# PantoMatrix/PantoMatrix

Hardware: NVIDIA H100
Metric: motion_frames_per_sec (higher is better)
Workload: dtype fp16x3 (two fp16 operand planes, 3 products, f32 accumulate)

## Files before the change

### include/pm_emage.h

```cpp
#ifndef PM_EMAGE_H
#define PM_EMAGE_H
#include <stdint.h>
#ifdef __cplusplus
extern "C" {
#endif

#define PM_ABI_VERSION 5
#define PM_FMT_F16 0x100
int pm_abi_version(void);
int pm_memset_async(void* ptr, int value, long long bytes, void* stream);
int pm_device_cc(void);

int pm_tapgemm_f32(const float* A, long long a_bs, int lda, int batch, int rows_in, int cin,
                   const float* W, const float* bias, int taps, int stride, int pad,
                   int rows_out, int cout,
                   const float* residual, long long r_bs, int ldr,
                   int act, float slope,
                   float* out, long long o_bs, int ldo, void* stream);

int pm_tapgemm_tc(const uint16_t* A, long long a_ps, long long a_bs, int lda, int batch, int rows_in, int cin,
                  const uint16_t* W, long long w_ps, int w_rows, int ldw, int taps, int pad, int nsplit,
                  const float* bias, int rows_out, int cout,
                  const float* residual, long long r_bs, int ldr,
                  int act, int act_cols, float slope, float acc_scale,
                  float* out_f32, long long o_bs, int ldo,
                  uint16_t* out_bf16, long long ob_ps, long long ob_bs, int ldob, int out_nsplit,
                  const void* prefetch, long long prefetch_bytes, void* stream);

int pm_split_bf16(const float* x, long long x_bs, int ldx, int batch, int rows, int ch,
                  uint16_t* out, long long o_ps, long long o_bs, int ldo, int nsplit, void* stream);

int pm_wav_stem_f32(const float* audio, long long a_bs, long long a_ws, int batch, int windows, int n_samples,
                    const float* w1, const float* b1, const float* wd, const float* bd, int cout,
                    int ksize, int stride, int pad, int rows_out, float slope,
                    float* y1, float* sc,
                    uint16_t* planes, long long p_ps, int p_ld, int p_nsplit, void* stream);

int pm_add_layernorm_f32(const float* x, const float* r, const float* gamma, const float* beta,
                         float* out, long long rows, int ch, float eps,
                         uint16_t* planes, long long p_ps, int p_ld, int p_nsplit, void* stream);

int pm_attention_f32(const float* Q, int ldq, const float* K, int ldk, const float* V, int ldv,
                     float* O, int ldo, int batch, int heads, int tq, int tk, int head_dim,
                     uint16_t* planes, long long p_ps, int p_ld, int p_nsplit, void* stream);

int pm_attention_tc(const uint16_t* Q, long long q_ps, long long q_bs, int ldq, int q_cols, int q_col0,
                    const uint16_t* K, long long k_ps, long long k_bs, int ldk, int k_cols, int k_col0,
                    const uint16_t* V, long long v_ps, long long v_bs, int ldv, int v_cols, int v_col0,
                    float* O, int ldo, int batch, int heads, int tq, int tk, int head_dim,
                    uint16_t* planes, long long p_ps, int p_ld, int p_nsplit, void* stream);

int pm_add_rows_f32(const float* x, const float* pe, const float* spk, int first, int second,
                    float* out, int batch, int rows, int ch,
                    uint16_t* planes, long long p_ps, int p_ld, int p_nsplit, void* stream);
int pm_add2_f32(const float* a, const float* b, float* out, long long n, int ch,
                uint16_t* planes, long long p_ps, int p_ld, int p_nsplit, void* stream);
int pm_add2_strided_f32(const float* a, long long lda, const float* b, long long ldb, float* out, long long ldo,
                        long long rows, long long ch,
                        uint16_t* planes, long long p_ps, int p_ld, int p_nsplit, void* stream);

int pm_window_input_f32(const float* motion, const float* mask, const float* seed, const float* mask_embedding,
                        float* out, int batch, int total_len, int start, int win_len, int pre, int ch, long long seed_bs,
                        uint16_t* planes, long long p_ps, int p_ld, int p_nsplit, void* stream);

int pm_l2_argmin_f32(const float* z, long long rows, int rows_per_batch, long long z_bs,
                     const float* codebook, const float* e2, int n_codes, int e_dim, long long* index, void* stream);
int pm_l2_argmin_tc(const float* z, long long rows, int rows_per_batch, long long z_bs,
                    const float* codebook, const float* e2, int n_codes, int e_dim, long long* index, int max_ctas,
                    void* stream);
int pm_l2_argmin_simt_f32(const float* z, long long rows, int rows_per_batch, long long z_bs,
                          const float* codebook, const float* e2, int n_codes, int e_dim, long long* index, void* stream);
int pm_row_argmax_f32(const float* x, long long rows, int ch, int ldx, int rows_per_batch, long long x_bs,
                      long long* index, int* nonfinite, void* stream);
int pm_gather_rows_f32(const float* codebook, long long n_table, const long long* index, long long rows, int ch,
                       float* out, uint16_t* planes, long long p_ps, int p_ld, int p_nsplit, void* stream);
int pm_row_sqnorm_f32(const float* x, int rows, int ch, float* out, void* stream);

int pm_pose_compose_f32(const float* face, const float* upper, const float* hands, const float* lower,
                        float* expression, float* axis_angle, float* motion4inf, long long bt, void* stream);

int pm_global_trans_f32(const float* rec, int ld, int vel_off, const float* ref_trans, int ref_bs, float dt,
                        float* trans, int batch, int t, void* stream);

int pm_resample_poly_f32(const void* pcm, int is_int16, long long in_bs, int batch, long long n_in, int channels,
                         const float* bank, int up, int down, int taps, long long n_pre_remove,
                         float* out, long long out_bs, void* stream);

int pm_lstm_bidir_f32(const float* xproj, long long x_bs, int ldx, const float* whh,
                      float* y, long long y_bs, int ldy, unsigned int* barrier,
                      int batch, int t, int hidden, void* stream);
int pm_lstm_cond_f32(const float* spk, long long n_spk, int spk_dim, const long long* speaker_id,
// ... 11 lines not shown
```

### pantomatrix_b200/csrc/pm_tapgemm_tc.cu

```cuda
#include <cuda.h>
#include <stdio.h>
#include <stdlib.h>

#include <cstring>
#include "pm_common.cuh"
#include "../../include/pm_emage.h"


namespace {

constexpr int BM = 128;
constexpr int BK = 64;
constexpr int MMA_K = 16;
constexpr int A_TILE_BYTES = BM * BK * 2;
constexpr int CONSUMER_THREADS = 256;
constexpr int NUM_THREADS = CONSUMER_THREADS + 32;
constexpr int MAX_STAGES = 8;
constexpr int RING_KB = 200;

struct TcParams {
  int taps, pad, nsplit, kblocks;
  int rows_out, cout, batch;
  int R, NB;
  int w_rows;
  const float* bias;
  const float* residual; long long r_bs; int ldr;
  int act, act_cols; float slope;
  float* out_f32; long long o_bs; int ldo;
  __nv_bfloat16* out_bf16; long long ob_ps, ob_bs; int ldob; int out_nsplit;
  int stages;
  const uint8_t* prefetch; long long prefetch_bytes;
  float acc_scale;
};

#ifdef PM_TC_TIMING
__device__ unsigned long long pm_tc_stamps[4096 * 8];
#define PM_STAMP(i)                                                                                              \
  do {                                                                                                           \
    if ((threadIdx.x & 31) == 0) {                                                                               \
      const unsigned cta_ = (blockIdx.z * gridDim.y + blockIdx.y) * gridDim.x + blockIdx.x;                      \
      if (cta_ < 4096) pm_tc_stamps[cta_ * 8 + (i)] = (unsigned long long)clock64();                             \
    }                                                                                                            \
  } while (0)
#else
#define PM_STAMP(i) do {} while (0)
#endif

#include "pm_tc_ptx.cuh"

template <int BN, bool F16>
__device__ __forceinline__ void mma_k16(float (&d)[BN / 2], uint64_t a, uint64_t b) {
  static_assert(BN == 64, "64-column tiles (see pm_tapgemm_tc)");
  wgmma_m64n64k16<!F16>(d, a, b);
}

template <int BN, bool F16, int NSPLIT>
__device__ __forceinline__ void mma_kblock(float (&main)[BN / 2], float (&corr)[BN / 2], uint64_t a0, uint64_t w0) {
  constexpr uint64_t A_PL = A_TILE_BYTES >> 4, W_PL = (BN * BK * 2) >> 4, K_ST = (MMA_K * 2) >> 4;
  if constexpr (NSPLIT == 3) {
#pragma unroll
    for (int k = 0; k < BK / MMA_K; ++k) mma_k16<BN, F16>(corr, a0 + k * K_ST, w0 + 2 * W_PL + k * K_ST);
#pragma unroll
    for (int k = 0; k < BK / MMA_K; ++k) mma_k16<BN, F16>(corr, a0 + A_PL + k * K_ST, w0 + W_PL + k * K_ST);
#pragma unroll
    for (int k = 0; k < BK / MMA_K; ++k) mma_k16<BN, F16>(corr, a0 + 2 * A_PL + k * K_ST, w0 + k * K_ST);
  }
  if constexpr (NSPLIT >= 2) {
#pragma unroll
    for (int k = 0; k < BK / MMA_K; ++k) mma_k16<BN, F16>(corr, a0 + k * K_ST, w0 + W_PL + k * K_ST);
#pragma unroll
    for (int k = 0; k < BK / MMA_K; ++k) mma_k16<BN, F16>(corr, a0 + A_PL + k * K_ST, w0 + k * K_ST);
  }
#pragma unroll
  for (int k = 0; k < BK / MMA_K; ++k) mma_k16<BN, F16>(main, a0 + k * K_ST, w0 + k * K_ST);
}

template <int BN, bool F16, int NSPLIT>
__global__ void __launch_bounds__(NUM_THREADS, 1) tapgemm_tc_kernel(const __grid_constant__ CUtensorMap map_a,
                                                                  const __grid_constant__ CUtensorMap map_w,
                                                                  const TcParams p) {
  constexpr int W_TILE_BYTES = BN * BK * 2;
  constexpr int NACC = BN / 2;
  constexpr int ST = BN + 8;

  extern __shared__ __align__(1024) uint8_t smem_raw[];
  uint8_t* tiles = reinterpret_cast<uint8_t*>((reinterpret_cast<uintptr_t>(smem_raw) + 1023) & ~uintptr_t(1023));
  const int stage_bytes = p.nsplit * (A_TILE_BYTES + W_TILE_BYTES);
  const int ring_bytes = p.stages * stage_bytes > BM * ST * 4 ? p.stages * stage_bytes : BM * ST * 4;
  uint64_t* bars = reinterpret_cast<uint64_t*>(tiles + ring_bytes);
  uint64_t* full_bar = bars;
  uint64_t* empty_bar = bars + MAX_STAGES;

  const int warp = threadIdx.x >> 5, lane = threadIdx.x & 31;
  if (warp == 0) PM_STAMP(0);
  const int l0 = blockIdx.x * p.R;
  const int n0 = blockIdx.y * BN;
  const int b0 = blockIdx.z * p.NB;
  const int n_iter = p.taps * p.kblocks;

  if (threadIdx.x == CONSUMER_THREADS) {
    asm volatile("prefetch.tensormap [%0];" ::"l"(&map_a) : "memory");
    asm volatile("prefetch.tensormap [%0];" ::"l"(&map_w) : "memory");
    for (int s = 0; s < p.stages; ++s) {
      mbar_init(smem_u32(&full_bar[s]), 1);
      mbar_init(smem_u32(&empty_bar[s]), 2);
    }
    asm volatile("fence.mbarrier_init.release.cluster;" ::: "memory");
  }
  __syncthreads();
  if (warp == 0) PM_STAMP(1);

  if (warp == CONSUMER_THREADS / 32) {
    if (lane == 1 && p.prefetch) {
      const long long ncta = (long long)gridDim.x * gridDim.y * gridDim.z;
      const long long cta = ((long long)blockIdx.z * gridDim.y + blockIdx.y) * gridDim.x + blockIdx.x;
      long long share = ((p.prefetch_bytes + ncta - 1) / ncta + 127) & ~127LL;
      long long off = cta * share;
      long long end = off + share < p.prefetch_bytes ? off + share : p.prefetch_bytes;
      end &= ~15LL;
      for (; off < end; off += 16384) {
        const uint32_t n = (uint32_t)(end - off < 16384 ? end - off : 16384);
        asm volatile("cp.async.bulk.prefetch.L2.global [%0], %1;" ::"l"(p.prefetch + off), "r"(n) : "memory");
      }
    }
    __syncwarp();
    const uint32_t tx = (uint32_t)stage_bytes;
    int s = 0, tap = 0, kb = 0;
    uint32_t ph = 0;
    for (int it = 0; it < n_iter; ++it) {
      mbar_wait_fast(smem_u32(&empty_bar[s]), ph ^ 1u);
      if (elect_one()) {
        const uint32_t bar = smem_u32(&full_bar[s]);
        uint8_t* st = tiles + (size_t)s * stage_bytes;
        mbar_expect_tx(bar, tx);
        for (int pl = 0; pl < p.nsplit; ++pl) {
          tma_load_4d(smem_u32(st + pl * A_TILE_BYTES), &map_a, bar, kb * BK, l0 + tap - p.pad, b0, pl);
          tma_load_3d(smem_u32(st + p.nsplit * A_TILE_BYTES + pl * W_TILE_BYTES), &map_w, bar, kb * BK, tap * p.w_rows + n0, pl);
        }
      }
      __syncwarp();
      if (++s == p.stages) { s = 0; ph ^= 1u; }
      if (++kb == p.kblocks) { kb = 0; ++tap; }
    }
    return;
  }

  const int wg = threadIdx.x >> 7;
  float acc0[NACC], acc1[NACC], accc[NACC];
#pragma unroll
  for (int i = 0; i < NACC; ++i) { acc0[i] = 0.f; acc1[i] = 0.f; accc[i] = 0.f; }
  {
    const uint32_t tiles_u32 = smem_u32(tiles);
    int s = 0;
    uint32_t ph = 0;
    int prev = -1;
    auto kblock = [&](float (&main)[NACC]) {
      mbar_wait_fast(smem_u32(&full_bar[s]), ph);
      if (prev < 0 && warp == 0) PM_STAMP(2);
      const uint32_t a_base = tiles_u32 + (uint32_t)s * (uint32_t)stage_bytes + (uint32_t)wg * (64 * 128);
      const uint32_t w_base = tiles_u32 + (uint32_t)s * (uint32_t)stage_bytes + (uint32_t)(NSPLIT * A_TILE_BYTES);
      wgmma_fence();
      mma_kblock<BN, F16, NSPLIT>(main, accc, gmma_desc(GMMA_DESC_K_SW128, a_base), gmma_desc(GMMA_DESC_K_SW128, w_base));
      wgmma_commit();
      wgmma_wait<1>();
      if (prev >= 0 && threadIdx.x % 128 == 0) mbar_arrive(smem_u32(&empty_bar[prev]));
      prev = s;
      if (++s == p.stages) { s = 0; ph ^= 1u; }
    };
    int it = 0;
    for (; it + 1 < n_iter; it += 2) {
      kblock(acc0);
      kblock(acc1);
    }
    if (it < n_iter) kblock(acc0);
    if (warp == 0) PM_STAMP(3);
    wgmma_wait<0>();
    if (warp == 0) PM_STAMP(4);
    wgmma_fence_regs(acc0);
    wgmma_fence_regs(acc1);
    wgmma_fence_regs(accc);
  }
  named_bar_sync(1, CONSUMER_THREADS);
  {
    const int wq = (threadIdx.x >> 5) & 3, t4 = lane & 3;
    const int r0 = wg * 64 + wq * 16 + (lane >> 2);
    float* stg = reinterpret_cast<float*>(tiles);
#pragma unroll
    for (int i = 0; i < NACC / 4; ++i) {
      const int c = 8 * i + 2 * t4;
#pragma unroll
      for (int h = 0; h < 2; ++h) {
        float v0 = acc0[4 * i + 2 * h] + acc1[4 * i + 2 * h];
        float v1 = acc0[4 * i + 2 * h + 1] + acc1[4 * i + 2 * h + 1];
        v0 += accc[4 * i + 2 * h];
        v1 += accc[4 * i + 2 * h + 1];
        if constexpr (F16) { v0 *= p.acc_scale; v1 *= p.acc_scale; }
        *reinterpret_cast<float2*>(stg + (r0 + 8 * h) * ST + c) = make_float2(v0, v1);
      }
    }
  }
  named_bar_sync(1, CONSUMER_THREADS);

  const bool vec_f = p.out_f32 && ((p.ldo & 3) == 0) && ((reinterpret_cast<uintptr_t>(p.out_f32) & 15) == 0) && ((p.o_bs & 3) == 0);
  const bool vec_r = p.residual && ((p.ldr & 3) == 0) && ((reinterpret_cast<uintptr_t>(p.residual) & 15) == 0) && ((p.r_bs & 3) == 0);
  const bool vec_b = p.out_bf16 && ((p.ldob & 3) == 0) && ((reinterpret_cast<uintptr_t>(p.out_bf16) & 7) == 0) &&
                     ((p.ob_bs & 3) == 0) && ((p.ob_ps & 3) == 0);
  const bool all_vec = (!p.out_f32 || vec_f) && (!p.residual || vec_r) && (!p.out_bf16 || vec_b);
  const float act_slope = p.act == PM_ACT_NONE ? 1.f : (p.act == PM_ACT_RELU ? 0.f : p.slope);
  const int r_shift = 31 - __clz(p.R);
  constexpr int C4 = BN / 4;
  const float* stg = reinterpret_cast<const float*>(tiles);
#pragma unroll 1
  for (int item = threadIdx.x; item < BM * C4; item += CONSUMER_THREADS) {
    const int rt = item / C4, c = (item % C4) * 4;
    const int b = b0 + (rt >> r_shift), l = l0 + (rt & (p.R - 1));
    const int n = n0 + c;
    if (b >= p.batch || l >= p.rows_out || n >= p.cout) continue;
    const float4 x4 = *reinterpret_cast<const float4*>(stg + rt * ST + c);
    const long long of = (long long)b * p.o_bs + (long long)l * p.ldo;
    const long long orr = (long long)b * p.r_bs + (long long)l * p.ldr;
    const PmPlanes P{p.out_bf16 ? p.out_bf16 + (long long)b * p.ob_bs + (long long)l * p.ldob : nullptr,
                     p.ob_ps, p.ldob, p.out_nsplit};
    if (all_vec && n + 4 <= p.cout) {
      float4 x = x4;
      if (p.bias) { x.x += __ldg(p.bias + n); x.y += __ldg(p.bias + n + 1); x.z += __ldg(p.bias + n + 2); x.w += __ldg(p.bias + n + 3); }
      if (p.residual) {
        const float4 t = *reinterpret_cast<const float4*>(p.residual + orr + n);
        x.x += t.x; x.y += t.y; x.z += t.z; x.w += t.w;
      }
      x.x = x.x < 0.f ? (n < p.act_cols ? act_slope : 1.f) * x.x : x.x;
      x.y = x.y < 0.f ? (n + 1 < p.act_cols ? act_slope : 1.f) * x.y : x.y;
      x.z = x.z < 0.f ? (n + 2 < p.act_cols ? act_slope : 1.f) * x.z : x.z;
      x.w = x.w < 0.f ? (n + 3 < p.act_cols ? act_slope : 1.f) * x.w : x.w;
      if (p.out_f32) *reinterpret_cast<float4*>(p.out_f32 + of + n) = x;
      if (P.ptr) pm_store_planes4_t<F16>(P, 0, n, x);
    } else {
      const float xs[4] = {x4.x, x4.y, x4.z, x4.w};
#pragma unroll
      for (int k = 0; k < 4; ++k) {
        if (n + k >= p.cout) break;
        float y = xs[k];
        if (p.bias) y += __ldg(p.bias + n + k);
        if (p.residual) y += p.residual[orr + n + k];
        y = y < 0.f ? (n + k < p.act_cols ? act_slope : 1.f) * y : y;
        if (p.out_f32) p.out_f32[of + n + k] = y;
        if (P.ptr) pm_store_planes_t<F16>(P, 0, n + k, y);
      }
    }
  }
  if (warp == 0) PM_STAMP(5);
#ifdef PM_TC_TIMING
  named_bar_sync(1, CONSUMER_THREADS);
#endif
  if (warp == 0) PM_STAMP(6);
}

template <bool VEC, bool F16>
__global__ void __launch_bounds__(256) split_bf16_kernel(const float* __restrict__ x, long long x_bs, int ldx, int rows,
                                                         int ch, __nv_bfloat16* __restrict__ out, long long o_ps,
                                                         long long o_bs, int ldo, int nsplit) {
  const int b = blockIdx.y;
  const float* __restrict__ xb = x + (long long)b * x_bs;
  __nv_bfloat16* __restrict__ ob = out + (long long)b * o_bs;
  if (VEC) {
    const int ch4 = ch >> 2;
    const long long total = (long long)rows * ch4;
    for (long long i = (long long)blockIdx.x * blockDim.x + threadIdx.x; i < total; i += (long long)gridDim.x * blockDim.x) {
      const int r = (int)(i / ch4), c4 = (int)(i - (long long)r * ch4);
      const float4 v = *reinterpret_cast<const float4*>(xb + (long long)r * ldx + 4 * c4);
      const PmPlanes P{ob, o_ps, ldo, nsplit};
      pm_store_planes4_t<F16>(P, r, 4 * c4, v);
    }
  } else {
    const long long total = (long long)rows * ch;
    for (long long i = (long long)blockIdx.x * blockDim.x + threadIdx.x; i < total; i += (long long)gridDim.x * blockDim.x) {
      const int r = (int)(i / ch), c = (int)(i - (long long)r * ch);
      const PmPlanes P{ob, o_ps, ldo, nsplit};
      pm_store_planes_t<F16>(P, r, c, xb[(long long)r * ldx + c]);
    }
  }
}

template <int BN, bool F16, int NSPLIT>
int launch(const CUtensorMap& ma, const CUtensorMap& mw, TcParams& p, dim3 grid, cudaStream_t st) {
  const int stage_bytes = p.nsplit * (A_TILE_BYTES + BN * BK * 2);
  int stages = RING_KB * 1024 / stage_bytes;
  if (stages > MAX_STAGES) stages = MAX_STAGES;
  if (stages < 2) return PM_EUNSUPPORTED;
  p.stages = stages;
  const int staging = BM * (BN + 8) * 4;
  const size_t ring = (size_t)stages * stage_bytes > (size_t)staging ? (size_t)stages * stage_bytes : (size_t)staging;
  const size_t smem = ring + 1024  + 2 * MAX_STAGES * sizeof(uint64_t);
  static unsigned long long configured = 0;
  if (pm_first_use_on_device(configured)) {
    cudaError_t e = cudaFuncSetAttribute(tapgemm_tc_kernel<BN, F16, NSPLIT>, cudaFuncAttributeMaxDynamicSharedMemorySize, 227 * 1024);
    if (e != cudaSuccess) { configured = 0; return (int)e; }
  }
  tapgemm_tc_kernel<BN, F16, NSPLIT><<<grid, NUM_THREADS, smem, st>>>(ma, mw, p);
  PM_LAUNCH_CHECK();
}

}

extern "C" int pm_tapgemm_tc(const uint16_t* A, long long a_ps, long long a_bs, int lda, int batch, int rows_in, int cin,
                             const uint16_t* W, long long w_ps, int w_rows, int ldw, int taps, int pad, int nsplit,
                             const float* bias, int rows_out, int cout,
                             const float* residual, long long r_bs, int ldr,
                             int act, int act_cols, float slope, float acc_scale,
                             float* out_f32, long long o_bs, int ldo,
                             uint16_t* out_bf16, long long ob_ps, long long ob_bs, int ldob, int out_nsplit,
                             const void* prefetch, long long prefetch_bytes, void* stream) {
  PM_REQUIRE(A && W && (out_f32 || out_bf16));
  PM_TAKE_FMT(nsplit, f16);
  PM_TAKE_FMT(out_nsplit, out_f16);
  PM_REQUIRE(!out_bf16 || out_f16 == f16);
  PM_REQUIRE(f16 || acc_scale == 1.0f);
  PM_REQUIRE(!prefetch || (prefetch_bytes >= 0 && (reinterpret_cast<uintptr_t>(prefetch) & 15) == 0));
  PM_REQUIRE(batch > 0 && rows_in > 0 && rows_out > 0 && cin > 0 && cout > 0 && taps > 0);
  PM_REQUIRE(nsplit >= 1 && nsplit <= 3 && (!out_bf16 || (out_nsplit >= 1 && out_nsplit <= 3)));
  PM_REQUIRE(act >= PM_ACT_NONE && act <= PM_ACT_LEAKY);
  PM_REQUIRE((reinterpret_cast<uintptr_t>(A) & 15) == 0 && (reinterpret_cast<uintptr_t>(W) & 15) == 0);
  PM_REQUIRE((lda & 7) == 0 && (ldw & 7) == 0 && lda >= cin && ldw >= cin && w_rows >= cout);
  PM_REQUIRE(batch == 1 || (a_bs & 7) == 0);
  PM_REQUIRE(nsplit == 1 || ((a_ps & 7) == 0 && (w_ps & 7) == 0));
  PM_REQUIRE(!out_f32 || ldo >= cout);
  PM_REQUIRE(!out_bf16 || ldob >= cout);
  PM_REQUIRE(!residual || ldr >= cout);

  int R = 128;
  if (rows_out <= 64 && batch > 1) { R = 16; while (R < rows_out) R <<= 1; }
  const int NB = 128 / R;
  constexpr int BNsel = 64;
  PM_REQUIRE(w_rows % BNsel == 0);

  TcParams p;
  p.taps = taps; p.pad = pad; p.nsplit = nsplit; p.kblocks = (cin + BK - 1) / BK;
  p.rows_out = rows_out; p.cout = cout; p.batch = batch; p.R = R; p.NB = NB; p.w_rows = w_rows;
  p.bias = bias; p.residual = residual; p.r_bs = r_bs; p.ldr = ldr;
  p.act = act; p.act_cols = act_cols <= 0 ? cout : act_cols; p.slope = slope;
  p.out_f32 = out_f32; p.o_bs = o_bs; p.ldo = ldo;
  p.out_bf16 = reinterpret_cast<__nv_bfloat16*>(out_bf16); p.ob_ps = ob_ps; p.ob_bs = ob_bs; p.ldob = ldob;
  p.out_nsplit = out_bf16 ? out_nsplit : 0;
  p.stages = 0;
  p.prefetch = static_cast<const uint8_t*>(prefetch);
  p.prefetch_bytes = prefetch ? prefetch_bytes : 0;
  p.acc_scale = acc_scale;
  CUtensorMap ma, mw;
  {
    const long long bs_el = batch > 1 ? a_bs : (long long)rows_in * lda;
    const long long ps_el = nsplit > 1 ? a_ps : bs_el * batch;
    cuuint64_t dims[4] = {(cuuint64_t)cin, (cuuint64_t)rows_in, (cuuint64_t)batch, (cuuint64_t)nsplit};
    cuuint64_t strides[3] = {(cuuint64_t)lda * 2, (cuuint64_t)bs_el * 2, (cuuint64_t)ps_el * 2};
    cuuint32_t box[4] = {(cuuint32_t)BK, (cuuint32_t)R, (cuuint32_t)NB, 1};
    if (!encode_map(&ma, A, 4, dims, strides, box, f16)) return PM_EBADARG;
  }
  {
    const long long ps_el = nsplit > 1 ? w_ps : (long long)taps * w_rows * ldw;
    cuuint64_t dims[3] = {(cuuint64_t)cin, (cuuint64_t)taps * w_rows, (cuuint64_t)nsplit};
    cuuint64_t strides[2] = {(cuuint64_t)ldw * 2, (cuuint64_t)ps_el * 2};
    cuuint32_t box[3] = {(cuuint32_t)BK, (cuuint32_t)BNsel, 1};
    if (!encode_map(&mw, W, 3, dims, strides, box, f16)) return PM_EBADARG;
  }
  dim3 grid(pm_cdiv(rows_out, R), pm_cdiv(cout, BNsel), pm_cdiv(batch, NB));
  PM_REQUIRE(grid.z <= 65535 && grid.y <= 65535);
  const cudaStream_t st = (cudaStream_t)stream;
  if (f16) {
    if (nsplit == 1) return launch<BNsel, true, 1>(ma, mw, p, grid, st);
    if (nsplit == 2) return launch<BNsel, true, 2>(ma, mw, p, grid, st);
    return launch<BNsel, true, 3>(ma, mw, p, grid, st);
  }
  if (nsplit == 1) return launch<BNsel, false, 1>(ma, mw, p, grid, st);
  if (nsplit == 2) return launch<BNsel, false, 2>(ma, mw, p, grid, st);
  return launch<BNsel, false, 3>(ma, mw, p, grid, st);
}

#ifdef PM_TC_TIMING
extern "C" int pm_tc_timing_reset() {
  cudaError_t e = cudaDeviceSynchronize();
  if (e != cudaSuccess) return (int)e;
  void* d = nullptr;
  e = cudaGetSymbolAddress(&d, pm_tc_stamps);
  if (e != cudaSuccess) return (int)e;
  return (int)cudaMemset(d, 0, sizeof(unsigned long long) * 4096 * 8);
}
extern "C" int pm_tc_timing_read(unsigned long long* host) {
  cudaError_t e = cudaDeviceSynchronize();
  if (e != cudaSuccess) return (int)e;
  return (int)cudaMemcpyFromSymbol(host, pm_tc_stamps, sizeof(unsigned long long) * 4096 * 8);
}
#endif

extern "C" int pm_split_bf16(const float* x, long long x_bs, int ldx, int batch, int rows, int ch,
                             uint16_t* out, long long o_ps, long long o_bs, int ldo, int nsplit, void* stream) {
  PM_TAKE_FMT(nsplit, f16);
  PM_REQUIRE(x && out && batch >= 0 && rows >= 0 && ch > 0 && ldx >= ch && ldo >= ch && nsplit >= 1 && nsplit <= 3);
  if ((long long)batch * rows == 0) return PM_OK;
  PM_REQUIRE(batch <= 65535);
  const bool vec = (ch & 3) == 0 && (ldx & 3) == 0 && (x_bs & 3) == 0 && (ldo & 3) == 0 && (o_bs & 3) == 0 &&
                   (o_ps & 3) == 0 && (reinterpret_cast<uintptr_t>(x) & 15) == 0 && (reinterpret_cast<uintptr_t>(out) & 7) == 0;
  const long long work = (long long)rows * (vec ? ch / 4 : ch);
  long long gx = (work + 255) / 256;
  const long long cap = batch >= 132 * 4 ? 1 : (132 * 8 + batch - 1) / batch;
  if (gx > cap) gx = cap;
  dim3 grid((unsigned)gx, batch);
  __nv_bfloat16* o = reinterpret_cast<__nv_bfloat16*>(out);
  cudaStream_t st = (cudaStream_t)stream;
  if (f16) {
    if (vec) split_bf16_kernel<true, true><<<grid, 256, 0, st>>>(x, x_bs, ldx, rows, ch, o, o_ps, o_bs, ldo, nsplit);
    else split_bf16_kernel<false, true><<<grid, 256, 0, st>>>(x, x_bs, ldx, rows, ch, o, o_ps, o_bs, ldo, nsplit);
  } else {
    if (vec) split_bf16_kernel<true, false><<<grid, 256, 0, st>>>(x, x_bs, ldx, rows, ch, o, o_ps, o_bs, ldo, nsplit);
    else split_bf16_kernel<false, false><<<grid, 256, 0, st>>>(x, x_bs, ldx, rows, ch, o, o_ps, o_bs, ldo, nsplit);
  }
  PM_LAUNCH_CHECK();
}
```

### pantomatrix_b200/csrc/pm_tc_ptx.cuh

```cuda
#pragma once
#include <cuda.h>
#include <stdint.h>

__device__ __forceinline__ uint32_t smem_u32(const void* p) { return (uint32_t)__cvta_generic_to_shared(p); }

__device__ __forceinline__ void mbar_init(uint32_t bar, uint32_t count) {
  asm volatile("mbarrier.init.shared::cta.b64 [%0], %1;" ::"r"(bar), "r"(count) : "memory");
}
__device__ __forceinline__ void mbar_expect_tx(uint32_t bar, uint32_t bytes) {
  asm volatile("mbarrier.arrive.expect_tx.shared::cta.b64 _, [%0], %1;" ::"r"(bar), "r"(bytes) : "memory");
}
__device__ __forceinline__ void mbar_wait(uint32_t bar, uint32_t parity) {
  uint32_t spins = 0;
  long long t0 = 0;
  while (true) {
    uint32_t done;
    asm volatile(
        "{\n\t.reg .pred p;\n\t"
        "mbarrier.try_wait.parity.shared::cta.b64 p, [%1], %2;\n\t"
        "selp.u32 %0, 1, 0, p;\n\t}"
        : "=r"(done) : "r"(bar), "r"(parity) : "memory");
    if (done) return;
    if ((++spins & 0xFFFu) == 0) {
      const long long t = clock64();
      if (t0 == 0) t0 = t;
      else if (t - t0 > 4000000000LL) __trap();
    }
  }
}
template <int SLEEP_NS = 40>
__device__ __forceinline__ void mbar_wait_relaxed(uint32_t bar, uint32_t parity) {
  uint32_t spins = 0;
  while (true) {
    uint32_t done;
    asm volatile(
        "{\n\t.reg .pred p;\n\t"
        "mbarrier.try_wait.parity.shared::cta.b64 p, [%1], %2;\n\t"
        "selp.u32 %0, 1, 0, p;\n\t}"
        : "=r"(done) : "r"(bar), "r"(parity) : "memory");
    if (done) return;
    __nanosleep(SLEEP_NS);
    if (++spins > 50000000u) __trap();
  }
}
__device__ __forceinline__ void mbar_wait_fast(uint32_t bar, uint32_t parity) {
  uint32_t done;
  asm volatile(
      "{\n\t.reg .pred p;\n\t"
      "mbarrier.try_wait.parity.shared::cta.b64 p, [%1], %2;\n\t"
      "selp.u32 %0, 1, 0, p;\n\t}"
      : "=r"(done) : "r"(bar), "r"(parity) : "memory");
  if (!done) mbar_wait(bar, parity);
}
__device__ __forceinline__ bool elect_one() {
  uint32_t pred;
  asm volatile("{\n\t.reg .pred P1;\n\telect.sync _|P1, 0xffffffff;\n\tselp.u32 %0, 1, 0, P1;\n\t}" : "=r"(pred));
  return pred != 0;
}
__device__ __forceinline__ void tma_load_4d(uint32_t dst, const CUtensorMap* map, uint32_t bar, int c0, int c1, int c2, int c3) {
  asm volatile(
      "cp.async.bulk.tensor.4d.shared::cluster.global.mbarrier::complete_tx::bytes [%0], [%1, {%3, %4, %5, %6}], [%2];"
      ::"r"(dst), "l"(map), "r"(bar), "r"(c0), "r"(c1), "r"(c2), "r"(c3) : "memory");
}
__device__ __forceinline__ void tma_load_3d(uint32_t dst, const CUtensorMap* map, uint32_t bar, int c0, int c1, int c2) {
  asm volatile(
      "cp.async.bulk.tensor.3d.shared::cluster.global.mbarrier::complete_tx::bytes [%0], [%1, {%3, %4, %5}], [%2];"
      ::"r"(dst), "l"(map), "r"(bar), "r"(c0), "r"(c1), "r"(c2) : "memory");
}
__device__ __forceinline__ void sts128(uint32_t addr, float a, float b, float c, float d) {
  asm volatile("st.shared.v4.f32 [%0], {%1, %2, %3, %4};" ::"r"(addr), "f"(a), "f"(b), "f"(c), "f"(d) : "memory");
}
__device__ __forceinline__ float4 lds128(uint32_t addr) {
  float4 v;
  asm volatile("ld.shared.v4.f32 {%0, %1, %2, %3}, [%4];" : "=f"(v.x), "=f"(v.y), "=f"(v.z), "=f"(v.w) : "r"(addr) : "memory");
  return v;
}
__device__ __forceinline__ void mbar_arrive(uint32_t bar) {
  asm volatile("mbarrier.arrive.shared::cta.b64 _, [%0];" ::"r"(bar) : "memory");
}
__device__ __forceinline__ void fence_proxy_async_smem() { asm volatile("fence.proxy.async.shared::cta;" ::: "memory"); }
__device__ __forceinline__ float4 ldg_stream4(const float4* p) {
  float4 v;
  asm volatile("ld.global.nc.L1::no_allocate.v4.f32 {%0, %1, %2, %3}, [%4];"
               : "=f"(v.x), "=f"(v.y), "=f"(v.z), "=f"(v.w) : "l"(p));
  return v;
}
__device__ __forceinline__ void named_bar_sync(uint32_t id, uint32_t threads) {
  asm volatile("bar.sync %0, %1;" ::"r"(id), "r"(threads) : "memory");
}

__device__ __forceinline__ void wgmma_fence() { asm volatile("wgmma.fence.sync.aligned;" ::: "memory"); }
__device__ __forceinline__ void wgmma_commit() { asm volatile("wgmma.commit_group.sync.aligned;" ::: "memory"); }
template <int N>
__device__ __forceinline__ void wgmma_wait() { asm volatile("wgmma.wait_group.sync.aligned %0;" ::"n"(N) : "memory"); }
template <int R>
__device__ __forceinline__ void wgmma_fence_regs(float (&d)[R]) {
#pragma unroll
  for (int i = 0; i < R; ++i) asm volatile("" : "+f"(d[i])::"memory");
}
constexpr uint64_t GMMA_DESC_K_SW128 = (1ull << 62) | ((uint64_t)(1024 >> 4) << 32) | (1ull << 16);
constexpr uint64_t gmma_desc_mn_sw128(uint32_t lbo_bytes) {
  return (1ull << 62) | ((uint64_t)(1024 >> 4) << 32) | ((uint64_t)(lbo_bytes >> 4) << 16);
}
__device__ __forceinline__ uint64_t gmma_desc(uint64_t hi, uint32_t smem_addr) { return hi | (uint64_t)((smem_addr >> 4) & 0x3FFFu); }

#define PM_D8(i) "+f"(d[i]), "+f"(d[i + 1]), "+f"(d[i + 2]), "+f"(d[i + 3]), "+f"(d[i + 4]), "+f"(d[i + 5]), "+f"(d[i + 6]), "+f"(d[i + 7])
#define PM_WGMMA_N64(TY)                                                                                   \
  asm volatile("{\n\t.reg .pred p;\n\tsetp.ne.b32 p, %34, 0;\n\t"                                           \
               "wgmma.mma_async.sync.aligned.m64n64k16.f32." TY "." TY " {%0, %1, %2, %3, %4, %5, %6, %7, %8, %9, %10, %11, %12, %13, %14, %15, %16, %17, %18, %19, %20, %21, %22, %23, %24, %25, %26, %27, %28, %29, %30, %31}, %32, %33, p, 1, 1, 0, %35;\n\t}" \
               : PM_D8(0), PM_D8(8), PM_D8(16), PM_D8(24) \
               : "l"(da), "l"(db), "r"(1), "n"(TRANS_B))
template <bool BF16, int TRANS_B = 0>
__device__ __forceinline__ void wgmma_m64n64k16(float (&d)[32], uint64_t da, uint64_t db) {
  if constexpr (BF16) PM_WGMMA_N64("bf16");
  else PM_WGMMA_N64("f16");
}
#undef PM_WGMMA_N64
#define PM_WGMMA_N192(TY)                                                                                   \
  asm volatile("{\n\t.reg .pred p;\n\tsetp.ne.b32 p, %98, 0;\n\t"                                           \
               "wgmma.mma_async.sync.aligned.m64n192k16.f32." TY "." TY " {%0, %1, %2, %3, %4, %5, %6, %7, %8, %9, %10, %11, %12, %13, %14, %15, %16, %17, %18, %19, %20, %21, %22, %23, %24, %25, %26, %27, %28, %29, %30, %31, %32, %33, %34, %35, %36, %37, %38, %39, %40, %41, %42, %43, %44, %45, %46, %47, %48, %49, %50, %51, %52, %53, %54, %55, %56, %57, %58, %59, %60, %61, %62, %63, %64, %65, %66, %67, %68, %69, %70, %71, %72, %73, %74, %75, %76, %77, %78, %79, %80, %81, %82, %83, %84, %85, %86, %87, %88, %89, %90, %91, %92, %93, %94, %95}, %96, %97, p, 1, 1, 0, %99;\n\t}" \
               : PM_D8(0), PM_D8(8), PM_D8(16), PM_D8(24), PM_D8(32), PM_D8(40), PM_D8(48), PM_D8(56), PM_D8(64), PM_D8(72), PM_D8(80), PM_D8(88) \
               : "l"(da), "l"(db), "r"(1), "n"(TRANS_B))
template <bool BF16, int TRANS_B = 0>
__device__ __forceinline__ void wgmma_m64n192k16(float (&d)[96], uint64_t da, uint64_t db) {
  if constexpr (BF16) PM_WGMMA_N192("bf16");
  else PM_WGMMA_N192("f16");
}
#undef PM_WGMMA_N192
#define PM_WGMMA_N256(TY)                                                                                   \
  asm volatile("{\n\t.reg .pred p;\n\tsetp.ne.b32 p, %130, 0;\n\t"                                           \
               "wgmma.mma_async.sync.aligned.m64n256k16.f32." TY "." TY " {%0, %1, %2, %3, %4, %5, %6, %7, %8, %9, %10, %11, %12, %13, %14, %15, %16, %17, %18, %19, %20, %21, %22, %23, %24, %25, %26, %27, %28, %29, %30, %31, %32, %33, %34, %35, %36, %37, %38, %39, %40, %41, %42, %43, %44, %45, %46, %47, %48, %49, %50, %51, %52, %53, %54, %55, %56, %57, %58, %59, %60, %61, %62, %63, %64, %65, %66, %67, %68, %69, %70, %71, %72, %73, %74, %75, %76, %77, %78, %79, %80, %81, %82, %83, %84, %85, %86, %87, %88, %89, %90, %91, %92, %93, %94, %95, %96, %97, %98, %99, %100, %101, %102, %103, %104, %105, %106, %107, %108, %109, %110, %111, %112, %113, %114, %115, %116, %117, %118, %119, %120, %121, %122, %123, %124, %125, %126, %127}, %128, %129, p, 1, 1, 0, %131;\n\t}" \
               : PM_D8(0), PM_D8(8), PM_D8(16), PM_D8(24), PM_D8(32), PM_D8(40), PM_D8(48), PM_D8(56), PM_D8(64), PM_D8(72), PM_D8(80), PM_D8(88), PM_D8(96), PM_D8(104), PM_D8(112), PM_D8(120) \
               : "l"(da), "l"(db), "r"(1), "n"(TRANS_B))
template <bool BF16, int TRANS_B = 0>
__device__ __forceinline__ void wgmma_m64n256k16(float (&d)[128], uint64_t da, uint64_t db) {
  if constexpr (BF16) PM_WGMMA_N256("bf16");
  else PM_WGMMA_N256("f16");
}
#undef PM_WGMMA_N256
#undef PM_D8

typedef CUresult (*EncodeTiledFn)(CUtensorMap*, CUtensorMapDataType, cuuint32_t, void*, const cuuint64_t*,
                                  const cuuint64_t*, const cuuint32_t*, const cuuint32_t*, CUtensorMapInterleave,
                                  CUtensorMapSwizzle, CUtensorMapL2promotion, CUtensorMapFloatOOBfill);

static inline EncodeTiledFn get_encode() {
  static EncodeTiledFn fn = nullptr;
  if (!fn) {
    void* sym = nullptr;
    cudaDriverEntryPointQueryResult q;
    if (cudaGetDriverEntryPoint("cuTensorMapEncodeTiled", &sym, cudaEnableDefault, &q) == cudaSuccess &&
        q == cudaDriverEntryPointSuccess)
      fn = reinterpret_cast<EncodeTiledFn>(sym);
  }
  return fn;
}

static inline bool encode_map(CUtensorMap* m, const void* base, int rank, const cuuint64_t* dims, const cuuint64_t* strides_bytes,
                const cuuint32_t* box, bool f16 = false) {
  EncodeTiledFn fn = get_encode();
  if (!fn) return false;
  cuuint32_t ones[5] = {1, 1, 1, 1, 1};
  return fn(m, f16 ? CU_TENSOR_MAP_DATA_TYPE_FLOAT16 : CU_TENSOR_MAP_DATA_TYPE_BFLOAT16, (cuuint32_t)rank,
            const_cast<void*>(base), dims, strides_bytes, box, ones, CU_TENSOR_MAP_INTERLEAVE_NONE,
            CU_TENSOR_MAP_SWIZZLE_128B, CU_TENSOR_MAP_L2_PROMOTION_L2_256B,
            CU_TENSOR_MAP_FLOAT_OOB_FILL_NONE) == CUDA_SUCCESS;
}
```

### pantomatrix_b200/ops.py

```python
from __future__ import annotations

import math

import torch

from . import _lib

ACT_NONE, ACT_RELU, ACT_LEAKY = 0, 1, 2
ROW_NONE, ROW_PE, ROW_SPK = 0, 1, 2

launch_count = 0

FMT_F16 = 0x100
F16_ACT_SCALE = 64.0
_PLANE_DTYPE = torch.bfloat16


def set_plane_format(name: str) -> None:
    global _PLANE_DTYPE
    _PLANE_DTYPE = {"bf16": torch.bfloat16, "fp16": torch.float16}[name]


def plane_format() -> str:
    return "fp16" if _PLANE_DTYPE == torch.float16 else "bf16"


def _fmt_bit(t) -> int:
    return FMT_F16 if t.dtype == torch.float16 else 0


def _stream() -> int:
    return torch.cuda.current_stream().cuda_stream


def _ptr(t) -> int | None:
    return None if t is None else t.data_ptr()


def _chk(t: torch.Tensor, dtype=torch.float32):
    if not t.is_cuda:
        raise _lib.PmError("pantomatrix_b200 ops need CUDA tensors (no CPU fallback)")
    if t.dtype != dtype:
        raise _lib.PmError(f"expected {dtype}, got {t.dtype}")
    if t.dim() and t.stride(-1) != 1 and t.shape[-1] != 1:
        raise _lib.PmError("innermost dimension must be contiguous")
    return t


def _call(name, *args):
    global launch_count
    launch_count += 1
    _lib.call(name, *args)


def _bs_ld(t: torch.Tensor):
    return (t.stride(0) if t.shape[0] > 1 else t.shape[1] * t.stride(1)), t.stride(1)


def tapgemm(a, w, bias, *, rows_out=None, stride=1, pad=0, act=ACT_NONE, slope=0.0, residual=None, out=None):
    _chk(a), _chk(w)
    batch, rows_in, cin = a.shape
    taps, cout, cin_w = w.shape
    assert cin_w == cin and w.is_contiguous(), (w.shape, a.shape)
    if rows_out is None:
        rows_out = (rows_in + 2 * pad - taps) // stride + 1
    if out is None:
        out = torch.empty(batch, rows_out, cout, device=a.device, dtype=torch.float32)
    else:
        assert out.shape == (batch, rows_out, cout), (out.shape, (batch, rows_out, cout))
    _chk(out)
    if residual is not None:
        _chk(residual)
        assert residual.shape == out.shape
    if (taps == 1 and pad == 0 and stride == 1 and batch > 1 and a.stride(0) == rows_in * a.stride(1)
            and out.stride(0) == rows_out * out.stride(1)
            and (residual is None or residual.stride(0) == rows_out * residual.stride(1))):
        a = a.reshape(1, batch * rows_in, cin) if a.is_contiguous() else a.as_strided(
            (1, batch * rows_in, cin), (0, a.stride(1), 1), a.storage_offset())
        flat = lambda t: t.as_strided((1, batch * rows_out, cout), (0, t.stride(1), 1), t.storage_offset())
        out_v = flat(out)
        res_v = flat(residual) if residual is not None else None
        batch_k, rows_in_k, rows_out_k = 1, batch * rows_in, batch * rows_out
    else:
        out_v, res_v, batch_k, rows_in_k, rows_out_k = out, residual, batch, rows_in, rows_out
    a_bs, lda = _bs_ld(a)
    o_bs, ldo = _bs_ld(out_v)
    r_bs, ldr = _bs_ld(res_v) if res_v is not None else (0, 0)
    _call("pm_tapgemm_f32", a.data_ptr(), a_bs, lda, batch_k, rows_in_k, cin,
          w.data_ptr(), _ptr(bias), taps, stride, pad, rows_out_k, cout,
          _ptr(res_v), r_bs, ldr, act, float(slope), out_v.data_ptr(), o_bs, ldo, _stream())
    return out


def wav_stem(audio, a_bs, a_ws, batch, windows, n_samples, w1, b1, wd, bd, *, stride, pad, slope, offset=0, nsplit=0):
    _chk(audio)
    cout, ks = w1.shape
# ... 261 lines not shown
    expression = torch.empty(bs, t, 100, device=device, dtype=torch.float32)
    axis_angle = torch.empty(bs, t, 165, device=device, dtype=torch.float32)
    motion4inf = torch.empty(bs, t, 337, device=device, dtype=torch.float32)
    _call("pm_pose_compose_f32", _ptr(face), _ptr(upper), _ptr(hands), _ptr(lower), expression.data_ptr(),
          axis_angle.data_ptr(), motion4inf.data_ptr(), bs * t, _stream())
    return expression, axis_angle, motion4inf


def global_trans(rec, ref_trans, dt, vel_off=54):
    _chk(rec), _chk(ref_trans)
    assert rec.is_contiguous()
    bs, t, ld = rec.shape
    assert ref_trans.shape == (bs, 3)
    trans = torch.empty(bs, t, 3, device=rec.device, dtype=torch.float32)
    _call("pm_global_trans_f32", rec.data_ptr(), ld, vel_off, ref_trans.data_ptr(), ref_trans.stride(0), float(dt),
          trans.data_ptr(), bs, t, _stream())
    return trans




def _round_up(x, m):
    return (x + m - 1) // m * m


class Planes:
    __slots__ = ("t", "rows", "ch", "slack")

    def __init__(self, t, rows, ch, slack=0):
        self.t, self.rows, self.ch, self.slack = t, rows, ch, slack

    def flat(self):
        ns, b, r, ld = self.t.shape
        assert self.t.stride(1) == r * self.t.stride(2)
        return Planes(self.t.as_strided((ns, 1, b * r, ld), (self.t.stride(0), b * r * self.t.stride(2), self.t.stride(2), 1),
                                        self.t.storage_offset()), b * r, self.ch, self.slack)

    @property
    def nsplit(self):
        return self.t.shape[0]

    @property
    def batch(self):
        return self.t.shape[1]


def split_bf16(x, nsplit, slack_rows=0):
    _chk(x)
    batch, rows, ch = x.shape
    pl = _new_planes(nsplit, (batch, rows), ch, x.device, slack_rows)
    x_bs, ldx = _bs_ld(x)
    _call("pm_split_bf16", x.data_ptr(), x_bs, ldx, batch, rows, ch, pl.t.data_ptr(), pl.t.stride(0), pl.t.stride(1),
          pl.t.stride(2), nsplit | _fmt_bit(pl.t), _stream())
    return pl


class PackedW:
    __slots__ = ("t", "taps", "cout", "cin", "w_rows", "ldw", "acc_scale")

    def __init__(self, w, nsplit):
        taps, cout, cin = w.shape
        bn = 64 if cout <= 64 else 128
        self.taps, self.cout, self.cin = taps, cout, cin
        self.w_rows, self.ldw = _round_up(cout, bn), _round_up(cin, 8)
        full = torch.zeros(taps, self.w_rows, self.ldw, device=w.device, dtype=torch.float32)
        full[:, :cout, :cin] = w
        self.acc_scale = 1.0
        if _PLANE_DTYPE == torch.float16:
            m = float(full.abs().max())
            if m > 0.0 and math.isfinite(m):
                k = math.floor(math.log2(32768.0 / m))
                full = full * (2.0 ** k)
                self.acc_scale = 2.0 ** -k
            self.acc_scale /= F16_ACT_SCALE
        planes, rem = [], full
        for _ in range(nsplit):
            p = rem.to(_PLANE_DTYPE)
            planes.append(p)
            rem = rem - p.float()
        self.t = torch.stack(planes).contiguous()


def tapgemm_tc(a: Planes, w: PackedW, bias, *, rows_in=None, rows_out, pad=0, act=ACT_NONE, act_cols=0, slope=0.0,
               residual=None, want_f32=True, out_nsplit=0, out=None, a_view=None, out_slack=0, prefetch=None):
    t = a.t
    nsplit, batch = t.shape[0], t.shape[1]
    assert nsplit == w.t.shape[0] and t.dtype == w.t.dtype, "A and W must use the same split and plane format"
    fmt = _fmt_bit(t)
    rows_a, cin, lda = (a.rows, a.ch, t.stride(2)) if a_view is None else a_view
    if rows_in is not None:
        rows_a = rows_in
    assert cin == w.cin, (cin, w.cin)
    cout = w.cout
    dev = t.device
    out_f = None
    if want_f32:
        out_f = out if out is not None else torch.empty(batch, rows_out, cout, device=dev, dtype=torch.float32)
        assert out_f.shape == (batch, rows_out, cout)
    o_bs, ldo = _bs_ld(out_f) if out_f is not None else (0, 0)
    out_p = None
    if out_nsplit:
        out_p = _new_planes(out_nsplit, (batch, rows_out), cout, dev, out_slack, dtype=t.dtype)
    r_bs, ldr = _bs_ld(residual) if residual is not None else (0, 0)
    if residual is not None:
        _chk(residual)
        assert residual.shape == (batch, rows_out, cout)
    _call("pm_tapgemm_tc", t.data_ptr(), t.stride(0), t.stride(1), lda, batch, rows_a, cin,
          w.t.data_ptr(), w.t.stride(0), w.w_rows, w.ldw, w.taps, pad, nsplit | fmt,
          _ptr(bias), rows_out, cout, _ptr(residual), r_bs, ldr, act, act_cols, float(slope), float(w.acc_scale),
          _ptr(out_f), o_bs, ldo,
          None if out_p is None else out_p.t.data_ptr(), 0 if out_p is None else out_p.t.stride(0),
          0 if out_p is None else out_p.t.stride(1), 0 if out_p is None else out_p.t.stride(2),
          out_nsplit | (fmt if out_nsplit else 0),
          None if prefetch is None else prefetch.data_ptr(),
          0 if prefetch is None else prefetch.numel() * prefetch.element_size(), _stream())
    return out_f, out_p




def lstm_bidir(xproj, whh, barrier, hidden):
    _chk(xproj), _chk(whh)
    assert xproj.is_contiguous() and whh.is_contiguous() and whh.shape == (2, 4 * hidden, hidden)
    batch, t, w = xproj.shape
    assert w == 8 * hidden
    y = torch.empty(batch, t, 2 * hidden, device=xproj.device, dtype=torch.float32)
    _call("pm_lstm_bidir_f32", xproj.data_ptr(), xproj.stride(0), xproj.stride(1), whh.data_ptr(), y.data_ptr(),
          y.stride(0), y.stride(1), barrier.data_ptr(), batch, t, hidden, _stream())
    return y


def rot6d_to_aa(rot6d, slot, n_sel):
    _chk(rot6d)
    assert rot6d.is_contiguous() and rot6d.shape[-1] == n_sel * 6
    rows = rot6d.numel() // (n_sel * 6)
    out = torch.empty(*rot6d.shape[:-1], 165, device=rot6d.device, dtype=torch.float32)
    _call("pm_rot6d_to_aa_f32", rot6d.data_ptr(), rows, n_sel, slot.data_ptr(), out.data_ptr(), _stream())
    return out


def softmax2_mix(sel, c1, c2, out=None):
    _chk(sel), _chk(c1), _chk(c2)
    assert sel.is_contiguous() and c1.is_contiguous() and c2.is_contiguous() and sel.shape[-1] == 2
    ch = c1.shape[-1]
    rows = c1.numel() // ch
    if out is None:
        out = torch.empty_like(c1)
    _call("pm_softmax2_mix_f32", sel.data_ptr(), c1.data_ptr(), c2.data_ptr(), out.data_ptr(), rows, ch, out.stride(-2), _stream())
    return out
```

Before: 277,400.

## Add 128-column wgmma tiles with wave-based selection and setmaxnreg producer/consumer split

Adds a BN=128 tile path using wgmma m64n128k16 and picks 64 or 128 per launch from a wave-count heuristic over the SM count, or from an explicit tile hint passed in the nsplit word. The producer is widened to a full warpgroup that gives registers back with setmaxnreg, so the consumer warpgroups can hold the larger accumulators (three NACC arrays). The intent is more reuse of the A tile per CTA and fewer CTAs for wide cout layers. The risks are register pressure or spills at 232 registers with 3x64 accumulators, fewer CTAs per wave, and a device-attribute query on every call.

```diff
diff --git a/include/pm_emage.h b/include/pm_emage.h
--- a/include/pm_emage.h
+++ b/include/pm_emage.h
@@ -7,6 +7,7 @@
 
 #define PM_ABI_VERSION 5
 #define PM_FMT_F16 0x100
+#define PM_TC_TILE_SHIFT 16
 int pm_abi_version(void);
 int pm_memset_async(void* ptr, int value, long long bytes, void* stream);
 int pm_device_cc(void);
diff --git a/pantomatrix_b200/csrc/pm_tapgemm_tc.cu b/pantomatrix_b200/csrc/pm_tapgemm_tc.cu
--- a/pantomatrix_b200/csrc/pm_tapgemm_tc.cu
+++ b/pantomatrix_b200/csrc/pm_tapgemm_tc.cu
@@ -13,8 +13,13 @@
 constexpr int BK = 64;
 constexpr int MMA_K = 16;
 constexpr int A_TILE_BYTES = BM * BK * 2;
+constexpr int PRODUCER_THREADS = 128;
 constexpr int CONSUMER_THREADS = 256;
-constexpr int NUM_THREADS = CONSUMER_THREADS + 32;
+constexpr int NUM_THREADS = PRODUCER_THREADS + CONSUMER_THREADS;
+constexpr int PRODUCER_REGS = 40, CONSUMER_REGS = 232;
+static_assert(PRODUCER_THREADS * PRODUCER_REGS + CONSUMER_THREADS * CONSUMER_REGS == (65536 / NUM_THREADS & ~7) * NUM_THREADS,
+              "the setmaxnreg split must use exactly the launch's register pool");
+constexpr int STAMP_WARP = PRODUCER_THREADS / 32;
 constexpr int MAX_STAGES = 8;
 constexpr int RING_KB = 200;
 
@@ -50,8 +55,9 @@
 
 template <int BN, bool F16>
 __device__ __forceinline__ void mma_k16(float (&d)[BN / 2], uint64_t a, uint64_t b) {
-  static_assert(BN == 64, "64-column tiles (see pm_tapgemm_tc)");
-  wgmma_m64n64k16<!F16>(d, a, b);
+  static_assert(BN == 64 || BN == 128, "64- or 128-column tiles (see pm_tapgemm_tc)");
+  if constexpr (BN == 64) wgmma_m64n64k16<!F16>(d, a, b);
+  else wgmma_m64n128k16<!F16>(d, a, b);
 }
 
 template <int BN, bool F16, int NSPLIT>
@@ -92,13 +98,13 @@
   uint64_t* empty_bar = bars + MAX_STAGES;
 
   const int warp = threadIdx.x >> 5, lane = threadIdx.x & 31;
-  if (warp == 0) PM_STAMP(0);
+  if (warp == STAMP_WARP) PM_STAMP(0);
   const int l0 = blockIdx.x * p.R;
   const int n0 = blockIdx.y * BN;
   const int b0 = blockIdx.z * p.NB;
   const int n_iter = p.taps * p.kblocks;
 
-  if (threadIdx.x == CONSUMER_THREADS) {
+  if (threadIdx.x == 0) {
     asm volatile("prefetch.tensormap [%0];" ::"l"(&map_a) : "memory");
     asm volatile("prefetch.tensormap [%0];" ::"l"(&map_w) : "memory");
     for (int s = 0; s < p.stages; ++s) {
@@ -108,10 +114,11 @@
     asm volatile("fence.mbarrier_init.release.cluster;" ::: "memory");
   }
   __syncthreads();
-  if (warp == 0) PM_STAMP(1);
-
-  if (warp == CONSUMER_THREADS / 32) {
-    if (lane == 1 && p.prefetch) {
+  if (warp == STAMP_WARP) PM_STAMP(1);
+
+  if (warp < PRODUCER_THREADS / 32) {
+    setmaxnreg_dec<PRODUCER_REGS>();
+    if (warp == 1 && lane == 0 && p.prefetch) {
       const long long ncta = (long long)gridDim.x * gridDim.y * gridDim.z;
       const long long cta = ((long long)blockIdx.z * gridDim.y + blockIdx.y) * gridDim.x + blockIdx.x;
       long long share = ((p.prefetch_bytes + ncta - 1) / ncta + 127) & ~127LL;
@@ -123,7 +130,7 @@
         asm volatile("cp.async.bulk.prefetch.L2.global [%0], %1;" ::"l"(p.prefetch + off), "r"(n) : "memory");
       }
     }
-    __syncwarp();
+    if (warp != 0) return;
     const uint32_t tx = (uint32_t)stage_bytes;
     int s = 0, tap = 0, kb = 0;
     uint32_t ph = 0;
@@ -145,7 +152,9 @@
     return;
   }
 
-  const int wg = threadIdx.x >> 7;
+  setmaxnreg_inc<CONSUMER_REGS>();
+  const int ct = threadIdx.x - PRODUCER_THREADS;
+  const int wg = ct >> 7;
   float acc0[NACC], acc1[NACC], accc[NACC];
 #pragma unroll
   for (int i = 0; i < NACC; ++i) { acc0[i] = 0.f; acc1[i] = 0.f; accc[i] = 0.f; }
@@ -156,14 +165,14 @@
     int prev = -1;
     auto kblock = [&](float (&main)[NACC]) {
       mbar_wait_fast(smem_u32(&full_bar[s]), ph);
-      if (prev < 0 && warp == 0) PM_STAMP(2);
+      if (prev < 0 && warp == STAMP_WARP) PM_STAMP(2);
       const uint32_t a_base = tiles_u32 + (uint32_t)s * (uint32_t)stage_bytes + (uint32_t)wg * (64 * 128);
       const uint32_t w_base = tiles_u32 + (uint32_t)s * (uint32_t)stage_bytes + (uint32_t)(NSPLIT * A_TILE_BYTES);
       wgmma_fence();
       mma_kblock<BN, F16, NSPLIT>(main, accc, gmma_desc(GMMA_DESC_K_SW128, a_base), gmma_desc(GMMA_DESC_K_SW128, w_base));
       wgmma_commit();
       wgmma_wait<1>();
-      if (prev >= 0 && threadIdx.x % 128 == 0) mbar_arrive(smem_u32(&empty_bar[prev]));
+      if (prev >= 0 && ct % 128 == 0) mbar_arrive(smem_u32(&empty_bar[prev]));
       prev = s;
       if (++s == p.stages) { s = 0; ph ^= 1u; }
     };
@@ -173,16 +182,16 @@
       kblock(acc1);
     }
     if (it < n_iter) kblock(acc0);
-    if (warp == 0) PM_STAMP(3);
+    if (warp == STAMP_WARP) PM_STAMP(3);
     wgmma_wait<0>();
-    if (warp == 0) PM_STAMP(4);
+    if (warp == STAMP_WARP) PM_STAMP(4);
     wgmma_fence_regs(acc0);
     wgmma_fence_regs(acc1);
     wgmma_fence_regs(accc);
   }
   named_bar_sync(1, CONSUMER_THREADS);
   {
-    const int wq = (threadIdx.x >> 5) & 3, t4 = lane & 3;
+    const int wq = warp & 3, t4 = lane & 3;
     const int r0 = wg * 64 + wq * 16 + (lane >> 2);
     float* stg = reinterpret_cast<float*>(tiles);
 #pragma unroll
@@ -211,7 +220,7 @@
   constexpr int C4 = BN / 4;
   const float* stg = reinterpret_cast<const float*>(tiles);
 #pragma unroll 1
-  for (int item = threadIdx.x; item < BM * C4; item += CONSUMER_THREADS) {
+  for (int item = ct; item < BM * C4; item += CONSUMER_THREADS) {
     const int rt = item / C4, c = (item % C4) * 4;
     const int b = b0 + (rt >> r_shift), l = l0 + (rt & (p.R - 1));
     const int n = n0 + c;
@@ -248,11 +257,11 @@
       }
     }
   }
-  if (warp == 0) PM_STAMP(5);
+  if (warp == STAMP_WARP) PM_STAMP(5);
 #ifdef PM_TC_TIMING
   named_bar_sync(1, CONSUMER_THREADS);
 #endif
-  if (warp == 0) PM_STAMP(6);
+  if (warp == STAMP_WARP) PM_STAMP(6);
 }
 
 template <bool VEC, bool F16>
@@ -300,6 +309,25 @@
   PM_LAUNCH_CHECK();
 }
 
+template <int BN>
+int launch_fmt(const CUtensorMap& ma, const CUtensorMap& mw, TcParams& p, dim3 grid, cudaStream_t st, bool f16) {
+  if (f16) {
+    if (p.nsplit == 1) return launch<BN, true, 1>(ma, mw, p, grid, st);
+    if (p.nsplit == 2) return launch<BN, true, 2>(ma, mw, p, grid, st);
+    return launch<BN, true, 3>(ma, mw, p, grid, st);
+  }
+  if (p.nsplit == 1) return launch<BN, false, 1>(ma, mw, p, grid, st);
+  if (p.nsplit == 2) return launch<BN, false, 2>(ma, mw, p, grid, st);
+  return launch<BN, false, 3>(ma, mw, p, grid, st);
+}
+
+int pick_bn(long long row_tiles, int cout, int w_rows, int sms) {
+  if (cout <= 64 || w_rows % 128) return 64;
+  const long long waves64 = (row_tiles * pm_cdiv(cout, 64) + sms - 1) / sms;
+  const long long waves128 = (row_tiles * pm_cdiv(cout, 128) + sms - 1) / sms;
+  return waves128 * 14 <= waves64 * 10 ? 128 : 64;
+}
+
 }
 
 extern "C" int pm_tapgemm_tc(const uint16_t* A, long long a_ps, long long a_bs, int lda, int batch, int rows_in, int cin,
@@ -311,6 +339,7 @@
                              uint16_t* out_bf16, long long ob_ps, long long ob_bs, int ldob, int out_nsplit,
                              const void* prefetch, long long prefetch_bytes, void* stream) {
   PM_REQUIRE(A && W && (out_f32 || out_bf16));
+  const int tile = (nsplit >> PM_TC_TILE_SHIFT) & 0xff;
   PM_TAKE_FMT(nsplit, f16);
   PM_TAKE_FMT(out_nsplit, out_f16);
   PM_REQUIRE(!out_bf16 || out_f16 == f16);
@@ -330,8 +359,15 @@
   int R = 128;
   if (rows_out <= 64 && batch > 1) { R = 16; while (R < rows_out) R <<= 1; }
   const int NB = 128 / R;
-  constexpr int BNsel = 64;
-  PM_REQUIRE(w_rows % BNsel == 0);
+  PM_REQUIRE(tile <= 2 && w_rows % 64 == 0 && (tile != 2 || w_rows % 128 == 0));
+  int BNsel = tile == 1 ? 64 : 128;
+  if (tile == 0) {
+    int dev = 0, sms = 0;
+    cudaError_t e = cudaGetDevice(&dev);
+    if (e == cudaSuccess) e = cudaDeviceGetAttribute(&sms, cudaDevAttrMultiProcessorCount, dev);
+    if (e != cudaSuccess) return (int)e;
+    BNsel = pick_bn((long long)pm_cdiv(rows_out, R) * pm_cdiv(batch, NB), cout, w_rows, sms);
+  }
 
   TcParams p;
   p.taps = taps; p.pad = pad; p.nsplit = nsplit; p.kblocks = (cin + BK - 1) / BK;
@@ -364,14 +400,8 @@
   dim3 grid(pm_cdiv(rows_out, R), pm_cdiv(cout, BNsel), pm_cdiv(batch, NB));
   PM_REQUIRE(grid.z <= 65535 && grid.y <= 65535);
   const cudaStream_t st = (cudaStream_t)stream;
-  if (f16) {
-    if (nsplit == 1) return launch<BNsel, true, 1>(ma, mw, p, grid, st);
-    if (nsplit == 2) return launch<BNsel, true, 2>(ma, mw, p, grid, st);
-    return launch<BNsel, true, 3>(ma, mw, p, grid, st);
-  }
-  if (nsplit == 1) return launch<BNsel, false, 1>(ma, mw, p, grid, st);
-  if (nsplit == 2) return launch<BNsel, false, 2>(ma, mw, p, grid, st);
-  return launch<BNsel, false, 3>(ma, mw, p, grid, st);
+  if (BNsel == 128) return launch_fmt<128>(ma, mw, p, grid, st, f16);
+  return launch_fmt<64>(ma, mw, p, grid, st, f16);
 }
 
 #ifdef PM_TC_TIMING
diff --git a/pantomatrix_b200/csrc/pm_tc_ptx.cuh b/pantomatrix_b200/csrc/pm_tc_ptx.cuh
--- a/pantomatrix_b200/csrc/pm_tc_ptx.cuh
+++ b/pantomatrix_b200/csrc/pm_tc_ptx.cuh
@@ -10,6 +10,7 @@
 __device__ __forceinline__ void mbar_expect_tx(uint32_t bar, uint32_t bytes) {
   asm volatile("mbarrier.arrive.expect_tx.shared::cta.b64 _, [%0], %1;" ::"r"(bar), "r"(bytes) : "memory");
 }
+static __device__ __noinline__ void pm_watchdog_trap() { __trap(); }
 __device__ __forceinline__ void mbar_wait(uint32_t bar, uint32_t parity) {
   uint32_t spins = 0;
   long long t0 = 0;
@@ -24,7 +25,7 @@
     if ((++spins & 0xFFFu) == 0) {
       const long long t = clock64();
       if (t0 == 0) t0 = t;
-      else if (t - t0 > 4000000000LL) __trap();
+      else if (t - t0 > 4000000000LL) pm_watchdog_trap();
     }
   }
 }
@@ -85,6 +86,10 @@
                : "=f"(v.x), "=f"(v.y), "=f"(v.z), "=f"(v.w) : "l"(p));
   return v;
 }
+template <int N>
+__device__ __forceinline__ void setmaxnreg_dec() { asm volatile("setmaxnreg.dec.sync.aligned.u32 %0;" ::"n"(N)); }
+template <int N>
+__device__ __forceinline__ void setmaxnreg_inc() { asm volatile("setmaxnreg.inc.sync.aligned.u32 %0;" ::"n"(N)); }
 __device__ __forceinline__ void named_bar_sync(uint32_t id, uint32_t threads) {
   asm volatile("bar.sync %0, %1;" ::"r"(id), "r"(threads) : "memory");
 }
@@ -116,7 +121,18 @@
   else PM_WGMMA_N64("f16");
 }
 #undef PM_WGMMA_N64
-#define PM_WGMMA_N192(TY)                                                                                   \
+#define PM_WGMMA_N128(TY)                                                                                   \
+  asm volatile("{\n\t.reg .pred p;\n\tsetp.ne.b32 p, %66, 0;\n\t"                                           \
+               "wgmma.mma_async.sync.aligned.m64n128k16.f32." TY "." TY " {%0, %1, %2, %3, %4, %5, %6, %7, %8, %9, %10, %11, %12, %13, %14, %15, %16, %17, %18, %19, %20, %21, %22, %23, %24, %25, %26, %27, %28, %29, %30, %31, %32, %33, %34, %35, %36, %37, %38, %39, %40, %41, %42, %43, %44, %45, %46, %47, %48, %49, %50, %51, %52, %53, %54, %55, %56, %57, %58, %59, %60, %61, %62, %63}, %64, %65, p, 1, 1, 0, %67;\n\t}" \
+               : PM_D8(0), PM_D8(8), PM_D8(16), PM_D8(24), PM_D8(32), PM_D8(40), PM_D8(48), PM_D8(56) \
+               : "l"(da), "l"(db), "r"(1), "n"(TRANS_B))
+template <bool BF16, int TRANS_B = 0>
+__device__ __forceinline__ void wgmma_m64n128k16(float (&d)[64], uint64_t da, uint64_t db) {
+  if constexpr (BF16) PM_WGMMA_N128("bf16");
+  else PM_WGMMA_N128("f16");
+}
+#undef PM_WGMMA_N128
+#define PM_WGMMA_N192(TY)                                                                                 \
   asm volatile("{\n\t.reg .pred p;\n\tsetp.ne.b32 p, %98, 0;\n\t"                                           \
                "wgmma.mma_async.sync.aligned.m64n192k16.f32." TY "." TY " {%0, %1, %2, %3, %4, %5, %6, %7, %8, %9, %10, %11, %12, %13, %14, %15, %16, %17, %18, %19, %20, %21, %22, %23, %24, %25, %26, %27, %28, %29, %30, %31, %32, %33, %34, %35, %36, %37, %38, %39, %40, %41, %42, %43, %44, %45, %46, %47, %48, %49, %50, %51, %52, %53, %54, %55, %56, %57, %58, %59, %60, %61, %62, %63, %64, %65, %66, %67, %68, %69, %70, %71, %72, %73, %74, %75, %76, %77, %78, %79, %80, %81, %82, %83, %84, %85, %86, %87, %88, %89, %90, %91, %92, %93, %94, %95}, %96, %97, p, 1, 1, 0, %99;\n\t}" \
                : PM_D8(0), PM_D8(8), PM_D8(16), PM_D8(24), PM_D8(32), PM_D8(40), PM_D8(48), PM_D8(56), PM_D8(64), PM_D8(72), PM_D8(80), PM_D8(88) \
diff --git a/pantomatrix_b200/ops.py b/pantomatrix_b200/ops.py
--- a/pantomatrix_b200/ops.py
+++ b/pantomatrix_b200/ops.py
@@ -12,6 +12,7 @@
 launch_count = 0
 
 FMT_F16 = 0x100
+TC_TILE_SHIFT = 16
 F16_ACT_SCALE = 64.0
 _PLANE_DTYPE = torch.bfloat16
 
@@ -439,7 +440,7 @@
 
 
 def tapgemm_tc(a: Planes, w: PackedW, bias, *, rows_in=None, rows_out, pad=0, act=ACT_NONE, act_cols=0, slope=0.0,
-               residual=None, want_f32=True, out_nsplit=0, out=None, a_view=None, out_slack=0, prefetch=None):
+               residual=None, want_f32=True, out_nsplit=0, out=None, a_view=None, out_slack=0, prefetch=None, tile=0):
     t = a.t
     nsplit, batch = t.shape[0], t.shape[1]
     assert nsplit == w.t.shape[0] and t.dtype == w.t.dtype, "A and W must use the same split and plane format"
@@ -448,6 +449,7 @@
     if rows_in is not None:
         rows_a = rows_in
     assert cin == w.cin, (cin, w.cin)
+    assert tile in (0, 64, 128), tile
     cout = w.cout
     dev = t.device
     out_f = None
@@ -463,7 +465,7 @@
         _chk(residual)
         assert residual.shape == (batch, rows_out, cout)
     _call("pm_tapgemm_tc", t.data_ptr(), t.stride(0), t.stride(1), lda, batch, rows_a, cin,
-          w.t.data_ptr(), w.t.stride(0), w.w_rows, w.ldw, w.taps, pad, nsplit | fmt,
+          w.t.data_ptr(), w.t.stride(0), w.w_rows, w.ldw, w.taps, pad, nsplit | fmt | (tile // 64) << TC_TILE_SHIFT,
           _ptr(bias), rows_out, cout, _ptr(residual), r_bs, ldr, act, act_cols, float(slope), float(w.acc_scale),
           _ptr(out_f), o_bs, ldo,
           None if out_p is None else out_p.t.data_ptr(), 0 if out_p is None else out_p.t.stride(0),
```

Measured after the change: 305,200 (median of 6 runs). +10.0%, better.
